# APRIL-ZJU/Ctrl-VIO

Hardware: AMD Instinct MI355X
Metric: sliding-window solves/sec (10 KF, 200 lm, 2000 IMU) (higher is better)
Workload: dtype f64; 1 GPU; config2: 10 KF / 200 landmarks / 2000 IMU sliding window (K = 24 knots, 814 reprojection blocks), <= 15 LM iterations (Ceres 1.14 trust region + projected line search); distinct_windows_per_gpu=64, streams_per_gpu=4, concurrent_solves_per_gpu=2

## Files before the change

### ctrl-vio_amd/csrc/factors.hpp

```cpp
#pragma once
#include "so3.hpp"

namespace ctv {

struct Knots4 {
  Q4 q[4];
  V3 p[4];
};

struct SegConst {
  V3 d[3];
  M3 JrI[3];
  CTV_DI M3 jri(int i) const { return JrI[i]; }
};
struct SegConstLazy {
  V3 d[3];
  const double *tab;
  CTV_DI M3 jri(int i) const {
    M3 J;
#pragma unroll
    for (int e = 0; e < 9; ++e) J.m[e] = tab[9 * i + e];
    return J;
  }
};
struct SegConstS {
  V3 d[3];
  M3 JrI[3];
  CTV_DI const M3 &jri(int i) const { return JrI[i]; }
};
CTV_DI void seg_const_lazy(const double *kd, const double *kjri, SegConstLazy &sc) {
#pragma unroll
  for (int i = 0; i < 3; ++i) sc.d[i] = mk(kd[3 * i], kd[3 * i + 1], kd[3 * i + 2]);
  sc.tab = kjri;
}
CTV_DI void seg_const(const Knots4 &k, SegConst &sc, bool want_jac) {
#pragma unroll
  for (int i = 0; i < 3; ++i) {
    sc.d[i] = so3_log(qmul(qconj(k.q[i]), k.q[i + 1]));
    if (want_jac) sc.JrI[i] = so3_Jr_inv(sc.d[i]);
  }
}

CTV_DI void knot_pair_const(const double *qa, const double *qb, double *d3, double *jri9) {
  const V3 dd = so3_log(qmul(qconj(qmk(qa[0], qa[1], qa[2], qa[3])), qmk(qb[0], qb[1], qb[2], qb[3])));
  d3[0] = dd.x; d3[1] = dd.y; d3[2] = dd.z;
  if (jri9) {
    const M3 J = so3_Jr_inv(mk(dd.x, dd.y, dd.z));
#pragma unroll
    for (int e = 0; e < 9; ++e) jri9[e] = J.m[e];
  }
}
CTV_DI void seg_const_load(const double *kd, const double *kjri, SegConst &sc, bool want_jac) {
#pragma unroll
  for (int i = 0; i < 3; ++i) {
    sc.d[i] = mk(kd[3 * i], kd[3 * i + 1], kd[3 * i + 2]);
    if (want_jac) {
#pragma unroll
      for (int e = 0; e < 9; ++e) sc.JrI[i].m[e] = kjri[9 * i + e];
    }
  }
}

struct ImuJac {
  M3 Jw[4], Ja[4];
  M3 Rinv_g;
  double lamA[4];
};

template <class SC> 
CTV_DI void imu_eval_core(const Knots4 &k, const SC &sc, double u, double idt, V3 gravity, const double bias[6],
                          const double gyro[3], const double acc[3], const double w[6], const M3 &RrefT, double r[6], bool want_jac, ImuJac &J) {
  double lamR[4], lamW[4];
  double (&lamA)[4] = J.lamA;
  basis<false, 2>(u, idt * idt, lamA);
  basis<true, 0>(u, 1.0, lamR);
  basis<true, 1>(u, idt, lamW);

  V3 accel = mk(0, 0, 0);
#pragma unroll
  for (int i = 0; i < 4; ++i) accel = accel + lamA[i] * k.p[i];

  Q4 Ainv[3], accq = qmk(0, 0, 0, 1);
  M3 Apost[4], JrK[3];
  Apost[3] = m3_id();
#pragma unroll
  for (int i = 2; i >= 0; --i) {
    const V3 nkd = (-lamR[i + 1]) * sc.d[i];
    Ainv[i] = so3_exp(nkd);
    accq = qmul_unit(accq, Ainv[i]);
    if (want_jac) { Apost[i] = q2R(accq); JrK[i] = so3_Jr(nkd); }
  }
  V3 om[4];
  om[0] = mk(0, 0, 0);
#pragma unroll
  for (int i = 0; i < 3; ++i) om[i + 1] = qrot(Ainv[i], om[i]) + lamW[i + 1] * sc.d[i];

  const Q4 Rinv_q = qmul_unit(accq, qconj(k.q[0]));
  const V3 ag = accel + gravity;
  const V3 a_pred = qrot(Rinv_q, ag);
  r[0] = w[0] * (om[3].x - (gyro[0] - bias[0]));
  r[1] = w[1] * (om[3].y - (gyro[1] - bias[1]));
  r[2] = w[2] * (om[3].z - (gyro[2] - bias[2]));
  r[3] = w[3] * (a_pred.x - (acc[0] - bias[3]));
  r[4] = w[4] * (a_pred.y - (acc[1] - bias[4]));
  r[5] = w[5] * (a_pred.z - (acc[2] - bias[5]));
  if (!want_jac) return;

  M3 (&Jw)[4] = J.Jw;
  M3 (&Ja)[4] = J.Ja;
#pragma unroll
  for (int i = 0; i < 4; ++i) { Jw[i] = m3_zero(); Ja[i] = m3_zero(); }
  {
    M3 dod = scale(Apost[1], lamW[1]);
#pragma unroll
    for (int i = 0; i < 3; ++i) {
      if (i > 0) dod = add(scale(mul(mul_hat(Apost[i], om[i]), JrK[i]), lamR[i + 1]), scale(Apost[i + 1], lamW[i + 1]));
      const M3 JrIi = sc.jri(i);
      Jw[i] = sub(Jw[i], mulT(dod, JrIi));
      Jw[i + 1] = add(Jw[i + 1], mul(dod, JrIi));
    }
  }
  const M3 Rinv = q2R(Rinv_q);
  J.Rinv_g = mul(Rinv, RrefT);
  {
    const M3 lhs = mul_hat(Rinv, ag);
    M3 Racc = q2R(k.q[0]);
    Ja[0] = add(Ja[0], mul(lhs, Racc));
#pragma unroll
    for (int i = 0; i < 3; ++i) {
      if (i > 0) Racc = mulT(Racc, q2R(Ainv[i - 1]));
      const M3 dad = scale(mul(mul(lhs, Racc), JrK[i]), lamR[i + 1]);
      const M3 JrIi = sc.jri(i);
      Ja[i] = sub(Ja[i], mulT(dad, JrIi));
      Ja[i + 1] = add(Ja[i + 1], mul(dad, JrIi));
    }
  }
}

CTV_DI void imu_row_gyro2(const M3 (&Jw)[4], const double w[6], const double r[6], int a, double out[16]) {
#pragma unroll
  for (int kk = 0; kk < 4; ++kk)
#pragma unroll
    for (int b = 0; b < 3; ++b) out[3 * kk + b] = w[a] * Jw[kk].m[3 * a + b];
  out[12] = out[13] = out[14] = 0.0;
  out[12 + a] = w[a];
  out[15] = r[a];
}

struct ImuMid3 {
  M3 Apost[3];
  M3 JrK[3];
  V3 om1, om2;
  V3 b[3];
  double lamR[4], lamW[4], lamA[4];
};
template <class SC> 
CTV_DI void imu_eval_values3(const double *gc, const SC &sc, double u, double idt, const double gyro[3], const double acc[3], const double w[6], double r[6], ImuMid3 &md) {
  basis<false, 2>(u, idt * idt, md.lamA);
  basis<true, 0>(u, 1.0, md.lamR);
  basis<true, 1>(u, idt, md.lamW);
  V3 ag = mk(gc[21], gc[22], gc[23]);
#pragma unroll
  for (int i = 1; i < 4; ++i) ag = ag + md.lamA[i] * mk(gc[3 * i], gc[3 * i + 1], gc[3 * i + 2]);
  Q4 Ainv[3], accq;
#pragma unroll
  for (int i = 2; i >= 0; --i) {
    const V3 nkd = (-md.lamR[i + 1]) * sc.d[i];
    Ainv[i] = so3_exp_small(nkd);
    accq = i == 2 ? Ainv[2] : qmul_unit(accq, Ainv[i]);
    md.Apost[i] = q2R(accq);
    md.JrK[i] = so3_Jr_small(nkd);
  }
  V3 om3;
  md.om1 = md.lamW[1] * sc.d[0];
  md.om2 = qrot(Ainv[1], md.om1) + md.lamW[2] * sc.d[1];
  om3 = qrot(Ainv[2], md.om2) + md.lamW[3] * sc.d[2];
  md.b[0] = mk(gc[12] * ag.x + gc[13] * ag.y + gc[14] * ag.z, gc[15] * ag.x + gc[16] * ag.y + gc[17] * ag.z,
                  gc[18] * ag.x + gc[19] * ag.y + gc[20] * ag.z);
  md.b[1] = qrot(Ainv[0], md.b[0]);
  md.b[2] = qrot(Ainv[1], md.b[1]);
  const V3 a_pred = qrot(Ainv[2], md.b[2]);
  r[0] = w[0] * (om3.x - (gyro[0] - gc[24]));
  r[1] = w[1] * (om3.y - (gyro[1] - gc[25]));
  r[2] = w[2] * (om3.z - (gyro[2] - gc[26]));
  r[3] = w[3] * (a_pred.x - (acc[0] - gc[27]));
  r[4] = w[4] * (a_pred.y - (acc[1] - gc[28]));
  r[5] = w[5] * (a_pred.z - (acc[2] - gc[29]));
}
template <class SC> CTV_DI void imu_apply_pair(const M3 &M, const SC &sc, int i, M3 &Ji, M3 &Ji1, bool first) {
  const M3 JrIi = sc.jri(i);
  const M3 A = mulT(M, JrIi), B = mul(M, JrIi);
#pragma unroll
  for (int e = 0; e < 9; ++e) { Ji.m[e] = first ? -A.m[e] : Ji.m[e] - A.m[e]; Ji1.m[e] = B.m[e]; }
}
template <class SC> CTV_DI void imu_jac_gyro3(const ImuMid3 &md, const SC &sc, M3 (&Jw)[4]) {
  imu_apply_pair(scale(md.Apost[1], md.lamW[1]), sc, 0, Jw[0], Jw[1], true);
  imu_apply_pair(add(scale(mul(mul_hat(md.Apost[1], md.om1), md.JrK[1]), md.lamR[2]), scale(md.Apost[2], md.lamW[2])), sc, 1, Jw[1], Jw[2], false);
  M3 dod = scale(mul(mul_hat(md.Apost[2], md.om2), md.JrK[2]), md.lamR[3]);
  dod.m[0] += md.lamW[3]; dod.m[4] += md.lamW[3]; dod.m[8] += md.lamW[3];
  imu_apply_pair(dod, sc, 2, Jw[2], Jw[3], false);
}
template <class SC> 
CTV_DI void imu_jac_accel3(const ImuMid3 &md, const SC &sc, const double *gc, M3 (&Ja)[4], M3 &Rinv_g) {
#pragma unroll
  for (int i = 0; i < 3; ++i)
#pragma unroll
    for (int j = 0; j < 3; ++j)
      Rinv_g.m[3 * i + j] = md.Apost[0].m[3 * i] * gc[12 + j] + md.Apost[0].m[3 * i + 1] * gc[15 + j] + md.Apost[0].m[3 * i + 2] * gc[18 + j];
  Ja[0] = mul_hat(md.Apost[0], md.b[0]);
#pragma unroll
  for (int i = 0; i < 3; ++i)
    imu_apply_pair(scale(mul(mul_hat(md.Apost[i], md.b[i]), md.JrK[i]), md.lamR[i + 1]), sc, i, Ja[i], Ja[i + 1], false);
}

CTV_DI void imu_row_accel3(const M3 (&Ja)[4], const double lamA[4], const M3 &Rinv_g, const double w[6], const double r[6], int a, double out[28]) {
#pragma unroll
  for (int kk = 0; kk < 4; ++kk)
#pragma unroll
    for (int b = 0; b < 3; ++b) {
      out[3 * kk + b] = w[3 + a] * Ja[kk].m[3 * a + b];
      out[16 + 3 * kk + b] = w[3 + a] * lamA[kk] * Rinv_g.m[3 * a + b];
    }
  out[12] = out[13] = out[14] = 0.0;
  out[12 + a] = w[3 + a];
  out[15] = r[3 + a];
}
template <class Sink> CTV_DI void imu_emit_cols(const ImuJac &J, const double w[6], Sink &sink) {
#pragma unroll
  for (int kk = 0; kk < 4; ++kk)
#pragma unroll
    for (int b = 0; b < 3; ++b) {
      double c6[6], p6[6];
#pragma unroll
      for (int a = 0; a < 3; ++a) {
        c6[a] = w[a] * J.Jw[kk].m[3 * a + b];
        c6[3 + a] = w[3 + a] * J.Ja[kk].m[3 * a + b];
        p6[a] = 0.0;
        p6[3 + a] = w[3 + a] * J.lamA[kk] * J.Rinv_g.m[3 * a + b];
      }
      sink.put_col(3 * kk + b, c6);
      sink.put_col(12 + 3 * kk + b, p6);
    }
#pragma unroll
  for (int a = 0; a < 3; ++a) {
    double g6[6] = {0.0, 0.0, 0.0, 0.0, 0.0, 0.0}, h6[6] = {0.0, 0.0, 0.0, 0.0, 0.0, 0.0};
    g6[a] = w[a];
    h6[3 + a] = w[3 + a];
    sink.put_col(24 + a, g6);
    sink.put_col(27 + a, h6);
  }
}
CTV_DI void imu_row_accel(const ImuJac &J, const double w[6], const double r[6], int a, double out[32]) {
#pragma unroll
  for (int kk = 0; kk < 4; ++kk)
#pragma unroll
    for (int b = 0; b < 3; ++b) {
      out[3 * kk + b] = w[3 + a] * J.Ja[kk].m[3 * a + b];
      out[12 + 3 * kk + b] = w[3 + a] * J.lamA[kk] * J.Rinv_g.m[3 * a + b];
    }
#pragma unroll
  for (int c = 24; c < 32; ++c) out[c] = 0.0;
  out[27 + a] = w[3 + a];
  out[30] = r[3 + a];
}
CTV_DI void imu_row_gyro(const ImuJac &J, const double w[6], const double r[6], int a, double out[16]) {
#pragma unroll
  for (int kk = 0; kk < 4; ++kk)
#pragma unroll
    for (int b = 0; b < 3; ++b) out[3 * kk + b] = w[a] * J.Jw[kk].m[3 * a + b];
  out[12] = out[13] = out[14] = 0.0;
  out[12 + a] = w[a];
  out[15] = r[a];
}

template <class Sink, class SC> 
CTV_DI void imu_eval(const Knots4 &k, const SC &sc, double u, double idt, V3 gravity, const double bias[6],
                     const double gyro[3], const double acc[3], const double w[6], const M3 &RrefT, double r[6], bool want_jac, Sink &sink) {
  ImuJac J;
  imu_eval_core<SC>(k, sc, u, idt, gravity, bias, gyro, acc, w, RrefT, r, want_jac, J);
  if (want_jac) imu_emit_cols(J, w, sink);
}

template <class SC, bool SMALL = false> CTV_DI Q4 eval_Rp(const Q4 q[4], const SC &sc, double u, M3 J[4], bool want_jac) {
  double c[4];
  basis<true, 0>(u, 1.0, c);
  Q4 accq = qmk(0, 0, 0, 1);
  M3 Apost[4], JrK[3];
  Apost[3] = m3_id();
#pragma unroll
  for (int i = 2; i >= 0; --i) {
    const V3 kd = c[i + 1] * sc.d[i];
    accq = qmul_unit(accq, so3_exp_sel<SMALL>(neg(kd)));
    if (want_jac) { JrK[i] = so3_Jr_sel<SMALL>(kd); Apost[i] = q2R(accq); }
  }
  const Q4 res = qmul_unit(q[0], qconj(accq));
  if (want_jac) {
    J[0] = Apost[0];
#pragma unroll
    for (int i = 0; i < 3; ++i) {
      const M3 Jh = scale(mul(Apost[i + 1], JrK[i]), c[i + 1]);
      J[i] = sub(J[i], mulT(Jh, sc.jri(i)));
      J[i + 1] = mul(Jh, sc.jri(i));
    }
  }
  return res;
}
template <class SC, bool SMALL = false> CTV_DI Q4 eval_RTp(const Q4 q[4], const SC &sc, double u, M3 J[4], bool want_jac) {
  double c[4];
  basis<true, 0>(u, 1.0, c);
  Q4 S[4];
  M3 JrK[3];
  S[0] = q[0];
#pragma unroll
  for (int i = 0; i < 3; ++i) {
    const V3 kd = c[i + 1] * sc.d[i];
    S[i + 1] = qmul_unit(S[i], so3_exp_sel<SMALL>(kd));
    if (want_jac) JrK[i] = so3_Jr_sel<SMALL>(neg(kd));
  }
  if (want_jac) {
    J[0] = q2R(S[0]);
#pragma unroll
    for (int i = 0; i < 3; ++i) {
      const M3 Jh = scale(mul(q2R(S[i]), JrK[i]), c[i + 1]);
      J[i] = sub(J[i], mulT(Jh, sc.jri(i)));
      J[i + 1] = mul(Jh, sc.jri(i));
    }
  }
  return qconj(S[3]);
}
template <class SC, bool SMALL = false> CTV_DI V3 eval_omega(const SC &sc, double u, double idt) {
  double c[4], dc[4];
  basis<true, 0>(u, 1.0, c);
  basis<true, 1>(u, idt, dc);
  V3 rv = dc[1] * sc.d[0];
#pragma unroll
  for (int i = 1; i < 3; ++i) rv = qrot(so3_exp_sel<SMALL>((-c[i + 1]) * sc.d[i]), rv) + dc[i + 1] * sc.d[i];
  return rv;
}
template <class SC> CTV_DI Q4 eval_R(const Q4 q[4], const SC &sc, double u) {
  double c[4];
  basis<true, 0>(u, 1.0, c);
  Q4 res = q[0];
#pragma unroll
  for (int i = 0; i < 3; ++i) res = qmul_unit(res, so3_exp(c[i + 1] * sc.d[i]));
  return res;
}

template <class SC> CTV_DI void pose_jac_T(const Q4 q[4], const SC &sc, double u, bool ext_on, Q4 q_SI, V3 p_SI, double *jt) {
  M3 J[4];
  const Q4 R = eval_Rp<SC>(q, sc, u, J, true);
  double c[4];
  basis<false, 0>(u, 1.0, c);
  M3 RSI = m3_id(), X = m3_zero();
  if (ext_on) { RSI = q2R(q_SI); X = scale(mul_hat(q2R(R), p_SI), -1.0); }
#pragma unroll
  for (int k = 0; k < 4; ++k) {
    const M3 B = mul(X, J[k]);
#pragma unroll
    for (int cc = 0; cc < 3; ++cc)
#pragma unroll
      for (int a = 0; a < 3; ++a) {
        jt[(6 * k + cc) * 6 + a] = ext_on ? RSI.m[a] * J[k].m[cc] + RSI.m[3 + a] * J[k].m[3 + cc] + RSI.m[6 + a] * J[k].m[6 + cc] : J[k].m[3 * a + cc];
        jt[(6 * k + cc) * 6 + 3 + a] = ext_on ? B.m[3 * a + cc] : 0.0;
        jt[(6 * k + 3 + cc) * 6 + a] = 0.0;
        jt[(6 * k + 3 + cc) * 6 + 3 + a] = a == cc ? c[k] : 0.0;
      }
  }
}

template <class SC> CTV_DI void nav_jac_T(const Q4 q[4], const SC &sc, double u, double idt, double *jt, double cv[4]) {
  pose_jac_T(q, sc, u, false, qmk(0.0, 0.0, 0.0, 1.0), mk(0.0, 0.0, 0.0), jt);
  basis<false, 1>(u, idt, cv);
}

CTV_DI void rel_pose_jac_T(Q4 q_a, V3 p_a, Q4 q_b, V3 p_b, double *jt_a, double *jt_b, Q4 &q_ab, V3 &p_ab) {
  q_ab = qmul(qconj(q_a), q_b);
  const M3 Ra = q2R(q_a), Rab = q2R(q_ab);
  const V3 d = p_b - p_a;
// ... 256 lines not shown
```

### ctrl-vio_amd/csrc/kernels_imu.hpp

```cpp
#pragma once

namespace ctv {

template <class T, int N> struct alignas(N * sizeof(T)) VecN { T v[N]; };

typedef double f64x4 __attribute__((ext_vector_type(4)));

__device__ __forceinline__ void imu_zero_share(const Dev &d, int mode, const ImuGroup &grp, int gidx, int zero_mode) {
  if (!zero_mode) return;
  const int w = grp.win, lane = threadIdx.x;
  const WinMeta &m = d.wins[w];
  const int tg = lin_target(d.lm[w], mode);
  double *Hpp = d.HppS[tg] + m.H0, *g = d.gS[tg] + m.u0;
  const int nH = m.P * m.ldh, first = (m.vis_lds && zero_mode == 1) ? 6 * m.K * m.ldh : 0;
  const int gi = gidx - m.grp0, per = (((nH - first) / 2 + m.ngrp - 1) / m.ngrp) * 2;
  const int lo = first + gi * per, hi = min(lo + per, nH);
  for (int i = lo + 2 * lane; i < hi; i += 128) *reinterpret_cast<double2 *>(Hpp + i) = double2{0.0, 0.0};
  if (gi == 0) {
    for (int i = lane; i < m.P; i += 64) g[i] = 0.0;
    if (lane == 0) { if (mode == LIN_SPEC) d.lm[w].cand_gmax_bits = 0ull; else d.lm[w].gmax_bits = 0ull; }
  }
}

__device__ __forceinline__ void imu_linearize_f64_body(const Dev &d, int mode, double *A , int gidx, int zero_mode) {
  const ImuGroup grp = d.groups[gidx];
  const int w = grp.win;
  if (!lin_run(d.lm[w], mode)) return;
  const bool jac = !lin_cost_only(d.lm[w], mode, d.prm);
  if (jac) imu_zero_share(d, mode, grp, gidx, zero_mode);
  const WinMeta &m = d.wins[w];
  const int lane = threadIdx.x, q4 = lane >> 4, l15 = lane & 15;
  const bool at_cand = mode == LIN_SPEC;
  double csum = 0.0;
  const double *s_quat = at_cand ? d.cquat : d.quat, *s_pos = at_cand ? d.cpos : d.pos, *s_bias = at_cand ? d.cbias : d.bias;
  Knots4 k;
  LocalFrame lf;
  lf.init(s_quat, s_pos, m.knot0 + grp.s);
  lf.load(s_quat, s_pos, m.knot0 + grp.s, k);
  const M3 RrefT = lf.RrefT();
  SegConstLazy sc;
  seg_const_lazy(d.lkd + 3 * (m.knot0 + grp.s), d.kjri + 9 * (m.knot0 + grp.s), sc);
  double bias[6], wgt[6];
  const double *bp = s_bias + 6 * (m.bias0 + grp.bias);
#pragma unroll
  for (int i = 0; i < 6; ++i) { bias[i] = bp[i]; wgt[i] = m.imu_w[i]; }
  const V3 grav = lf.rotate(m.gravity);
  const double idt = m.inv_dt;
  f64x4 acc00 = {0.0, 0.0, 0.0, 0.0}, acc10 = {0.0, 0.0, 0.0, 0.0}, acc11 = {0.0, 0.0, 0.0, 0.0}, gacc = {0.0, 0.0, 0.0, 0.0};
  const size_t Mt = (size_t)d.Mtot;
  if (!jac) {
    for (int c0 = 0; c0 < grp.count; c0 += 64) {
      const bool live = c0 + lane < grp.count;
      const int idx = m.imu0 + grp.start + min(c0 + lane, grp.count - 1);
      double gy[3], ac[3], r[6], wl[6];
#pragma unroll
      for (int i = 0; i < 3; ++i) { gy[i] = d.imu_meas[(size_t)i * Mt + idx]; ac[i] = d.imu_meas[(size_t)(3 + i) * Mt + idx]; }
#pragma unroll
      for (int i = 0; i < 6; ++i) wl[i] = live ? wgt[i] : 0.0;
      ImuJac J;
      imu_eval_core(k, sc, d.imu_u[idx], idt, grav, bias, gy, ac, wl, RrefT, r, false, J);
#pragma unroll
      for (int i = 0; i < 6; ++i) csum += 0.5 * r[i] * r[i];
    }
#pragma unroll
    for (int off = 32; off > 0; off >>= 1) csum += __shfl_xor(csum, off);
    if (lane == 0) d.imu_cost[gidx] = csum;
    return;
  }
  for (int c0 = 0; c0 < grp.count; c0 += 64) {
    const int nval = min(64, grp.count - c0);
    const bool live = lane < nval;
    const int idx = m.imu0 + grp.start + min(c0 + lane, grp.count - 1);
    double gy[3], ac[3], r[6];
#pragma unroll
    for (int i = 0; i < 3; ++i) { gy[i] = d.imu_meas[(size_t)i * Mt + idx]; ac[i] = d.imu_meas[(size_t)(3 + i) * Mt + idx]; }
    double wl[6];
#pragma unroll
    for (int i = 0; i < 6; ++i) wl[i] = live ? wgt[i] : 0.0;
    const int kmax = (nval + 3) & ~3;
    ImuJac J;
    imu_eval_core(k, sc, d.imu_u[idx], idt, grav, bias, gy, ac, wl, RrefT, r, true, J);
#pragma unroll
    for (int i = 0; i < 6; ++i) csum += 0.5 * r[i] * r[i];
#pragma unroll
    for (int a = 0; a < 3; ++a) {
      double row[32];
      imu_row_accel(J, wl, r, a, row);
      __builtin_amdgcn_wave_barrier();
#pragma unroll
      for (int c = 0; c < 32; ++c) A[lane * 33 + c] = row[c];
      lds_wave_sync();
      for (int k0 = 0; k0 < kmax; k0 += 4) {
        const double lo = A[(k0 + q4) * 33 + l15], hi = A[(k0 + q4) * 33 + 16 + l15];
        acc00 = __builtin_amdgcn_mfma_f64_16x16x4f64(lo, lo, acc00, 0, 0, 0);
        acc10 = __builtin_amdgcn_mfma_f64_16x16x4f64(hi, lo, acc10, 0, 0, 0);
        acc11 = __builtin_amdgcn_mfma_f64_16x16x4f64(hi, hi, acc11, 0, 0, 0);
      }
    }
#pragma unroll
    for (int a = 0; a < 3; ++a) {
      double row[16];
      imu_row_gyro(J, wl, r, a, row);
      __builtin_amdgcn_wave_barrier();
#pragma unroll
      for (int c = 0; c < 16; ++c) A[lane * 17 + c] = row[c];
      lds_wave_sync();
      for (int k0 = 0; k0 < kmax; k0 += 4) {
        const double v = A[(k0 + q4) * 17 + l15];
        gacc = __builtin_amdgcn_mfma_f64_16x16x4f64(v, v, gacc, 0, 0, 0);
      }
    }
  }
#pragma unroll
  for (int off = 32; off > 0; off >>= 1) csum += __shfl_xor(csum, off);
  if (lane == 0) d.imu_cost[gidx] = csum;
  __builtin_amdgcn_wave_barrier();
#pragma unroll
  for (int r = 0; r < 4; ++r) {
    const int row = q4 + 4 * r, col = l15;
    A[row * 32 + col] = acc00[r];
    A[(16 + row) * 32 + 16 + col] = acc11[r];
    A[(16 + row) * 32 + col] = acc10[r];
    A[col * 32 + 16 + row] = acc10[r];
  }
  lds_wave_sync();
  {
    const int tc = l15 < 12 ? l15 : (l15 < 15 ? l15 + 12 : 30);
#pragma unroll
    for (int r = 0; r < 4; ++r) {
      const int grow = q4 + 4 * r;
      const int tr = grow < 12 ? grow : (grow < 15 ? grow + 12 : 30);
      A[tr * 32 + tc] += gacc[r];
    }
  }
  lds_wave_sync();
  double *tile = d.imu_tiles + (size_t)gidx * 1024;
#pragma unroll
  for (int i = 0; i < 16; ++i) tile[i * 64 + lane] = A[i * 64 + lane];
}

typedef double f64x2 __attribute__((ext_vector_type(2)));
__device__ __forceinline__ void imu_chain_gyro(const double *A, int q4, int l15, int kmax, f64x4 &gacc) {
  unsigned addr = (unsigned)(size_t)(A + q4 * 17 + l15);
  double v0, v1;
  asm volatile("ds_read_b64 %0, %1" : "=v"(v0) : "v"(addr));
  for (int k0 = 0; k0 < kmax; k0 += 8) {
    asm volatile("ds_read_b64 %0, %1 offset:544" : "=v"(v1) : "v"(addr));
    asm volatile("s_waitcnt lgkmcnt(1)" : "+v"(v0));
    gacc = __builtin_amdgcn_mfma_f64_16x16x4f64(v0, v0, gacc, 0, 0, 0);
    addr += 8 * 17 * 8;
    asm volatile("ds_read_b64 %0, %1" : "=v"(v0) : "v"(addr));
    asm volatile("s_waitcnt lgkmcnt(1)" : "+v"(v1));
    gacc = __builtin_amdgcn_mfma_f64_16x16x4f64(v1, v1, gacc, 0, 0, 0);
  }
  asm volatile("s_waitcnt lgkmcnt(0)" : "+v"(v0));
}
__device__ __forceinline__ void imu_chain_accel(const double *A, int q4, int l15, int kmax, f64x4 &acc00, f64x4 &acc10) {
  unsigned addr = (unsigned)(size_t)(A + q4 * 33 + l15);
  f64x2 o0, o1;
  asm volatile("ds_read2_b64 %0, %1 offset1:16" : "=v"(o0) : "v"(addr));
  for (int k0 = 0; k0 < kmax; k0 += 8) {
    asm volatile("ds_read2_b64 %0, %1 offset0:132 offset1:148" : "=v"(o1) : "v"(addr));
    asm volatile("s_waitcnt lgkmcnt(1)" : "+v"(o0));
    acc00 = __builtin_amdgcn_mfma_f64_16x16x4f64(o0[0], o0[0], acc00, 0, 0, 0);
    acc10 = __builtin_amdgcn_mfma_f64_16x16x4f64(o0[1], o0[0], acc10, 0, 0, 0);
    addr += 8 * 33 * 8;
    asm volatile("ds_read2_b64 %0, %1 offset1:16" : "=v"(o0) : "v"(addr));
    asm volatile("s_waitcnt lgkmcnt(1)" : "+v"(o1));
    acc00 = __builtin_amdgcn_mfma_f64_16x16x4f64(o1[0], o1[0], acc00, 0, 0, 0);
    acc10 = __builtin_amdgcn_mfma_f64_16x16x4f64(o1[1], o1[0], acc10, 0, 0, 0);
  }
  asm volatile("s_waitcnt lgkmcnt(0)" : "+v"(o0));
}

__device__ __forceinline__ bool imu_fast_pred(const double kd[9], const double *imu_w) {
  double mx = 0.0;
#pragma unroll
  for (int i = 0; i < 3; ++i) mx = fmax(mx, __fma_rn(kd[3 * i + 2], kd[3 * i + 2], __fma_rn(kd[3 * i + 1], kd[3 * i + 1], __dmul_rn(kd[3 * i], kd[3 * i]))));
  return mx < 0.25 && imu_w[3] == imu_w[4] && imu_w[3] == imu_w[5];
}
struct ImuPre { double pc, kq; int fl; };
__device__ __forceinline__ void imu_prefetch(const Dev &d, int mode, const ImuGroup &g, int lane, ImuPre &o) {
  const bool at_cand = mode == LIN_SPEC;
  const double *s_quat = at_cand ? d.cquat : d.quat, *s_pos = at_cand ? d.cpos : d.pos, *s_bias = at_cand ? d.cbias : d.bias;
  const WinMeta &m = d.wins[g.win];
  const Lm &lm = d.lm[g.win];
  const double *kd = d.lkd + 3 * g.kabs, *kj = d.kjri + 9 * g.kabs;
  const double *q = s_quat + 4 * g.kabs, *pp = s_pos + 3 * g.kabs, *bp = s_bias + 6 * g.babs;
  o.pc = *(lane < 9 ? kd + lane : kj + (min(lane, 35) - 9));
  const double *src = lane < 4 ? q + lane : lane < 16 ? pp + (lane - 4) : lane < 21 ? q : lane < 24 ? m.gravity + (lane - 21)
                      : lane < 30 ? bp + (lane - 24) : lane < 36 ? m.imu_w + (lane - 30) : &m.inv_dt;
  o.kq = *src;
  const int32_t *fp = lane == 0 ? &lm.status : lane == 1 ? &lm.step_valid : lane == 2 ? &lm.iter : &lm.ls_active;
  o.fl = *fp;
}
__device__ __forceinline__ void imu_linearize_f64_fast(const Dev &d, int mode, double *A , int g0, int stride, int zero_mode) {
  const int lane = threadIdx.x, q4 = lane >> 4, l15 = lane & 15;
  const size_t Mt = (size_t)d.Mtot;
  int gidx = g0;
  ImuGroup grp = d.groups[gidx];
  ImuPre cur;
  imu_prefetch(d, mode, grp, lane, cur);
  double gyn[3], acn[3], un;
  {
    const int idx = grp.iabs + min(lane, grp.count - 1);
#pragma unroll
    for (int i = 0; i < 3; ++i) { gyn[i] = d.imu_meas[(size_t)i * Mt + idx]; acn[i] = d.imu_meas[(size_t)(3 + i) * Mt + idx]; }
    un = d.imu_u[idx];
  }
  bool has_next = gidx + stride < d.Gtot;
  ImuGroup grpn = d.groups[has_next ? gidx + stride : gidx];
  for (;;) {
  const bool has_next2 = has_next && gidx + 2 * stride < d.Gtot;
  const ImuGroup grpn2 = d.groups[has_next2 ? gidx + 2 * stride : gidx];
  ImuPre nxt;
  imu_prefetch(d, mode, grpn, lane, nxt);
  bool nmeas = false;
  do {
  const int w = grp.win;
  const int base = grp.iabs;
  SegConstS sc;
#pragma unroll
  for (int i = 0; i < 3; ++i) {
    sc.d[i] = mk(readlane_d(cur.pc, 3 * i), readlane_d(cur.pc, 3 * i + 1), readlane_d(cur.pc, 3 * i + 2));
#pragma unroll
    for (int e = 0; e < 9; ++e) sc.JrI[i].m[e] = readlane_d(cur.pc, 9 + 9 * i + e);
  }
  const int f_status = __builtin_amdgcn_readlane(cur.fl, 0), f_valid = __builtin_amdgcn_readlane(cur.fl, 1), f_iter = __builtin_amdgcn_readlane(cur.fl, 2),
            f_ls = __builtin_amdgcn_readlane(cur.fl, 3);
  if (!(f_status == 0 && (mode != LIN_SPEC || f_valid != 0))) break;
  const bool jac = !(mode == COST_AT_X || (mode == LIN_SPEC && f_iter >= d.prm.max_iters && f_ls == 0));
  {
    const double kd9[9] = {sc.d[0].x, sc.d[0].y, sc.d[0].z, sc.d[1].x, sc.d[1].y, sc.d[1].z, sc.d[2].x, sc.d[2].y, sc.d[2].z};
    const double w6[6] = {0.0, 0.0, 0.0, readlane_d(cur.kq, 33), readlane_d(cur.kq, 34), readlane_d(cur.kq, 35)};
    if (!imu_fast_pred(kd9, w6)) break;
  }
  long long *dbg = (d.dbg && gidx == 5000 && jac) ? d.dbg + 64 : nullptr;
  int dbi = 0;
  CTV_STAMP(dbg, dbi, 16, lane == 0);
  double *gc = A + 72 * 33;
  {
    double gcv = cur.kq;
    const M3 R0 = q2R(qmk(readlane_d(cur.kq, 0), readlane_d(cur.kq, 1), readlane_d(cur.kq, 2), readlane_d(cur.kq, 3)));
    const double pk = __shfl(cur.kq, 4 + min(lane, 11)), p0 = __shfl(cur.kq, 4 + min(lane, 11) % 3);
    if (lane < 12) gcv = pk - p0;
    else if (lane < 21) {
      const int e = lane - 12, src = 3 * (e % 3) + e / 3;
#pragma unroll
      for (int i = 0; i < 9; ++i) gcv = src == i ? R0.m[i] : gcv;
    }
    __builtin_amdgcn_wave_barrier();
    if (lane < 36) gc[lane] = gcv;
    lds_wave_sync();
  }
  const double idt = readlane_d(cur.kq, 36);
  double csum = 0.0;
  if (!jac) {
    for (int c0 = 0; c0 < grp.count; c0 += 64) {
      const bool live = c0 + lane < grp.count;
      const int idx = base + min(c0 + lane, grp.count - 1);
      double gy[3], ac[3], r[6], wl[6];
#pragma unroll
      for (int i = 0; i < 3; ++i) { gy[i] = d.imu_meas[(size_t)i * Mt + idx]; ac[i] = d.imu_meas[(size_t)(3 + i) * Mt + idx]; }
#pragma unroll
      for (int i = 0; i < 6; ++i) wl[i] = live ? gc[30 + i] : 0.0;
      ImuMid3 md;
      imu_eval_values3(gc, sc, d.imu_u[idx], idt, gy, ac, wl, r, md);
#pragma unroll
      for (int i = 0; i < 6; ++i) csum += 0.5 * r[i] * r[i];
    }
#pragma unroll
    for (int off = 32; off > 0; off >>= 1) csum += __shfl_xor(csum, off);
    if (lane == 0) d.imu_cost[gidx] = csum;
    break;
  }
  f64x4 acc00 = {0.0, 0.0, 0.0, 0.0}, acc10 = {0.0, 0.0, 0.0, 0.0}, gacc = {0.0, 0.0, 0.0, 0.0};
  double spp[10] = {0.0, 0.0, 0.0, 0.0, 0.0, 0.0, 0.0, 0.0, 0.0, 0.0};
  for (int c0 = 0; c0 < grp.count; c0 += 64) {
    CTV_STAMP(dbg, dbi, 16, lane == 0, csum);
    const int nval = min(64, grp.count - c0);
    const bool live = lane < nval;
    double gy[3], ac[3], r[6];
#pragma unroll
    for (int i = 0; i < 3; ++i) { gy[i] = gyn[i]; ac[i] = acn[i]; }
    const double u = un;
    {
      const bool last = c0 + 64 >= grp.count;
      const int idx = (last && has_next) ? grpn.iabs + min(lane, grpn.count - 1) : base + min(c0 + 64 + lane, grp.count - 1);
      nmeas = last;
#pragma unroll
      for (int i = 0; i < 3; ++i) { gyn[i] = d.imu_meas[(size_t)i * Mt + idx]; acn[i] = d.imu_meas[(size_t)(3 + i) * Mt + idx]; }
      un = d.imu_u[idx];
    }
    double wl[6];
#pragma unroll
    for (int i = 0; i < 6; ++i) wl[i] = live ? gc[30 + i] : 0.0;
    const int kmax = (nval + 3) & ~3;
    ImuMid3 md;
    imu_eval_values3(gc, sc, u, idt, gy, ac, wl, r, md);
#pragma unroll
    for (int i = 0; i < 6; ++i) csum += 0.5 * r[i] * r[i];
    CTV_STAMP(dbg, dbi, 16, lane == 0, csum);
    {
      M3 Jw[4];
      imu_jac_gyro3(md, sc, Jw);
      CTV_STAMP(dbg, dbi, 16, lane == 0, Jw[3].m[8]);
#pragma unroll
      for (int a = 0; a < 3; ++a) {
        double row[16];
        imu_row_gyro2(Jw, wl, r, a, row);
        __builtin_amdgcn_wave_barrier();
#pragma unroll
        for (int c = 0; c < 16; ++c) A[lane * 17 + c] = row[c];
        lds_wave_sync();
        imu_chain_gyro(A, q4, l15, kmax, gacc);
      }
    }
    CTV_STAMP(dbg, dbi, 16, lane == 0, gacc[0]);
    {
      M3 Ja[4], Rinv_g;
      imu_jac_accel3(md, sc, gc, Ja, Rinv_g);
      CTV_STAMP(dbg, dbi, 16, lane == 0, Ja[3].m[8] + Rinv_g.m[8]);
      {
        double la[4];
#pragma unroll
        for (int kk = 0; kk < 4; ++kk) la[kk] = wl[3] * md.lamA[kk];
        int e = 0;
#pragma unroll
        for (int ka = 0; ka < 4; ++ka)
#pragma unroll
          for (int kb = 0; kb <= ka; ++kb) { spp[e] += la[ka] * la[kb]; ++e; }
      }
#pragma unroll
      for (int a = 0; a < 3; ++a) {
        double row[28];
        imu_row_accel3(Ja, md.lamA, Rinv_g, wl, r, a, row);
        __builtin_amdgcn_wave_barrier();
#pragma unroll
        for (int c = 0; c < 28; ++c) A[lane * 33 + c] = row[c];
        lds_wave_sync();
        imu_chain_accel(A, q4, l15, kmax, acc00, acc10);
      }
    }
  }
  CTV_STAMP(dbg, dbi, 16, lane == 0, acc00[0] + acc10[0]);
  __builtin_amdgcn_wave_barrier();
#pragma unroll
  for (int i = 0; i < 16; ++i) A[i * 64 + lane] = 0.0;
  {
    double *S = A + 1024;
#pragma unroll
    for (int e = 0; e < 10; ++e) S[e * 64 + lane] = spp[e];
    S[10 * 64 + lane] = csum;
    lds_wave_sync();
    const int e = min(lane >> 2, 10), part = lane & 3;
    double t = 0.0;
#pragma unroll
    for (int i = 0; i < 16; ++i) t += S[e * 64 + part * 16 + i];
    t += __shfl_xor(t, 1);
    t += __shfl_xor(t, 2);
    __builtin_amdgcn_wave_barrier();
    if (lane < 40 && part == 0) S[704 + e] = t;
    if (lane == 40) d.imu_cost[gidx] = t;
  }
  lds_wave_sync();
  {
    const int c0 = l15 < 12 ? l15 : (l15 < 15 ? l15 + 15 : 30);
    const int cg = l15 < 12 ? l15 : (l15 < 15 ? l15 + 12 : 30);
    const bool cb = l15 >= 12 && l15 < 15;
#pragma unroll
    for (int r = 0; r < 4; ++r) {
      const int t = q4 + 4 * r;
      const int r0 = t < 12 ? t : (t < 15 ? t + 15 : 30), rg = t < 12 ? t : (t < 15 ? t + 12 : 30);
      const bool shared = !cb && !(t >= 12 && t < 15);
      A[r0 * 32 + c0] = shared ? acc00[r] + gacc[r] : acc00[r];
      if (!shared) A[rg * 32 + cg] = gacc[r];
      if (t < 12) { A[(12 + t) * 32 + c0] = acc10[r]; A[c0 * 32 + 12 + t] = acc10[r]; }
    }
    const int ka = lane / 12, kb = (lane / 3) & 3, b = lane % 3;
    const int hi = max(ka, kb), lo = min(ka, kb);
    if (lane < 48) A[(12 + 3 * ka + b) * 32 + 12 + 3 * kb + b] = A[1024 + 704 + hi * (hi + 1) / 2 + lo];
  }
  lds_wave_sync();
  double *tile = d.imu_tiles + (size_t)gidx * 1024;
#pragma unroll
  for (int i = 0; i < 8; ++i)
    *reinterpret_cast<double2 *>(tile + i * 128 + 2 * lane) = *reinterpret_cast<const double2 *>(A + i * 128 + 2 * lane);
  imu_zero_share(d, mode, grp, gidx, zero_mode);
  CTV_STAMP(dbg, dbi, 16, lane == 0);
  } while (false);
  if (!has_next) break;
  lds_wave_sync();
  if (!nmeas) {
    const int idx = grpn.iabs + min(lane, grpn.count - 1);
#pragma unroll
    for (int i = 0; i < 3; ++i) { gyn[i] = d.imu_meas[(size_t)i * Mt + idx]; acn[i] = d.imu_meas[(size_t)(3 + i) * Mt + idx]; }
    un = d.imu_u[idx];
  }
  gidx += stride;
  grp = grpn; grpn = grpn2; cur = nxt;
  has_next = has_next2;
  }
}

__device__ __forceinline__ bool imu_group_fast(const Dev &d, int gidx) {
  const ImuGroup grp = d.groups[gidx];
  const double *kd = d.lkd + 3 * grp.kabs;
  const double kd9[9] = {kd[0], kd[1], kd[2], kd[3], kd[4], kd[5], kd[6], kd[7], kd[8]};
  return imu_fast_pred(kd9, d.wins[grp.win].imu_w);
}
__global__ __launch_bounds__(64) __attribute__((amdgpu_waves_per_eu(1, 1))) void k_imu_linearize_f64(Dev d, int mode, int general_only, int zero_mode) {
  extern __shared__ __attribute__((aligned(32))) unsigned char smraw[];
  if (!general_only) imu_linearize_f64_fast(d, mode, reinterpret_cast<double *>(smraw), blockIdx.x, gridDim.x, zero_mode);
}
__device__ __forceinline__ void imu_rest_body(const Dev &d, int mode, int general_only, int zero_mode, unsigned char *smraw , int w) {
  const WinMeta &m = d.wins[w];
  for (int g0 = 0; g0 < m.ngrp; g0 += 64) {
    const int gl = g0 + (int)threadIdx.x;
    const bool need = gl < m.ngrp && (general_only || !imu_group_fast(d, m.grp0 + gl));
    unsigned long long todo = __ballot(need);
    while (todo) {
      const int b = __ffsll((long long)todo) - 1;
      todo &= todo - 1;
      imu_linearize_f64_body(d, mode, reinterpret_cast<double *>(smraw), m.grp0 + g0 + b, zero_mode);
      lds_wave_sync();
    }
  }
}
__global__ __launch_bounds__(64) __attribute__((amdgpu_waves_per_eu(1, 1))) void k_imu_linearize_rest(Dev d, int mode, int general_only, int zero_mode) {
  extern __shared__ __attribute__((aligned(32))) unsigned char smraw[];
  imu_rest_body(d, mode, general_only, zero_mode, smraw, blockIdx.x);
}

__device__ __forceinline__ int imu_knot_major_to_col(int j) {
  const int k = j / 6, c = j - 6 * k;
  return c < 3 ? 3 * k + c : 9 + 3 * k + c;
}
__device__ __forceinline__ void imu_bias_rows_accumulate(const Dev &d, const WinMeta &m, double *Hpp, double *g) {
  const int lane = threadIdx.x & 63, wave = threadIdx.x >> 6, ldh = m.ldh;
  const int nmine = (m.ngrp - wave + 3) >> 2;
  for (int i = lane; i < 195 * nmine; i += 64) {
    const int q = i / 195, t = i - 195 * q, gi = m.grp0 + wave + 4 * q;
    const ImuGroup grp = d.groups[gi];
    const double *tile = d.imu_tiles + (size_t)gi * 1024;
    const int B = 6 * grp.s, R = 6 * m.K + 6 * grp.bias;
    if (t < 144) {
      const int r = t / 24, j = t - 24 * r;
      atomicAdd(&Hpp[(long long)(R + r) * ldh + B + j], tile[(24 + r) * 32 + imu_knot_major_to_col(j)]);
    } else if (t < 165) {
      const int e = t - 144;
      const int r = e < 1 ? 0 : e < 3 ? 1 : e < 6 ? 2 : e < 10 ? 3 : e < 15 ? 4 : 5, c = e - r * (r + 1) / 2;
      atomicAdd(&Hpp[(long long)(R + r) * ldh + R + c], tile[(24 + r) * 32 + 24 + c]);
    } else {
      const int j = t - 165;
      atomicAdd(&g[j < 24 ? B + j : R + j - 24], tile[30 * 32 + (j < 24 ? imu_knot_major_to_col(j) : j)]);
    }
  }
}

__device__ __forceinline__ void assemble_imu_window(const Dev &d, int mode, int w, double *band ) {
  if (!lin_run(d.lm[w], mode) || lin_cost_only(d.lm[w], mode, d.prm)) return;
  const WinMeta &m = d.wins[w];
  const int K = m.K, ldh = m.ldh, tg = lin_target(d.lm[w], mode);
  double *Hpp = d.HppS[tg] + m.H0, *g = d.gS[tg] + m.u0;
  if (m.vis_lds) {
    imu_bias_rows_accumulate(d, m, Hpp, g);
    return;
  }
  if (band) {
    const int nb = 144 * K;
    for (int i = threadIdx.x; i < nb; i += 256) band[i] = 0.0;
    __syncthreads();
    for (int i = threadIdx.x; i < 300 * m.ngrp; i += 256) {
      const int gi = i / 300, t = i - 300 * gi;
      int a = (int)((sqrtf(8.0f * (float)t + 1.0f) - 1.0f) * 0.5f);
      a += ((a + 1) * (a + 2) / 2 <= t) ? 1 : 0;
      a -= (a * (a + 1) / 2 > t) ? 1 : 0;
      const int b = t - a * (a + 1) / 2;
      const ImuGroup grp = d.groups[m.grp0 + gi];
      const double v = d.imu_tiles[(size_t)(m.grp0 + gi) * 1024 + a * 32 + b];
      int ga = imu_col(a, grp.s, K, grp.bias), gb = imu_col(b, grp.s, K, grp.bias);
      if (ga < gb) { const int tmp = ga; ga = gb; gb = tmp; }
      const int k1 = ga / 6, k2 = gb / 6;
      atomicAdd(&band[((k2 * 4 + (k1 - k2)) * 6 + (ga - 6 * k1)) * 6 + (gb - 6 * k2)], v);
    }
    __syncthreads();
    for (int i = threadIdx.x; i < nb; i += 256) {
      const double v = band[i];
      if (v == 0.0) continue;
      const int r2 = i % 6, r1 = (i / 6) % 6, dk = (i / 36) % 4, k2 = i / 144;
      const int ga = 6 * (k2 + dk) + r1, gb = 6 * k2 + r2;
      atomicAdd(&Hpp[(long long)ga * ldh + gb], v);
    }
    imu_bias_rows_accumulate(d, m, Hpp, g);
    return;
  }
  for (int i = threadIdx.x; i < 31 * 30 * m.ngrp; i += 256) {
    const int gi = i / 930, e = i - 930 * gi;
    const ImuGroup grp = d.groups[m.grp0 + gi];
    const double *tile = d.imu_tiles + (size_t)(m.grp0 + gi) * 1024;
    const int b = e / 30, a = e % 30;
    const double v = tile[a * 32 + b];
    const int ga = imu_col(a, grp.s, K, grp.bias);
    if (b == 30) { atomicAdd(&g[ga], v); continue; }
    const int gb = imu_col(b, grp.s, K, grp.bias);
    if (ga >= gb) atomicAdd(&Hpp[(long long)ga * ldh + gb], v);
  }
}

}
```

Baseline: 50190 solves/s.

## Factor IMU Jacobian through shared pair-log transform and world-frame accel rows

Restructures the per-measurement IMU Jacobian so the knot-rotation chain rule (JrI pair terms) is applied once per group, as a 16x16 transform T on the accumulated Gram matrices, instead of per measurement. Accelerometer rows are rotated into a world frame, so the position block collapses to scalar lamA weights multiplied against a small 16-wide row using 4x4x4 MFMAs rather than a 28-wide row with a second 16x16 accumulator. This cuts per-sample ALU work and LDS traffic. In exchange it adds extra MFMA post-processing, more LDS scratch, and some numerical reordering in f64.

```diff
diff --git a/ctrl-vio_amd/csrc/factors.hpp b/ctrl-vio_amd/csrc/factors.hpp
--- a/ctrl-vio_amd/csrc/factors.hpp
+++ b/ctrl-vio_amd/csrc/factors.hpp
@@ -135,16 +135,6 @@
       Ja[i + 1] = add(Ja[i + 1], mul(dad, JrIi));
     }
   }
-}
-
-CTV_DI void imu_row_gyro2(const M3 (&Jw)[4], const double w[6], const double r[6], int a, double out[16]) {
-#pragma unroll
-  for (int kk = 0; kk < 4; ++kk)
-#pragma unroll
-    for (int b = 0; b < 3; ++b) out[3 * kk + b] = w[a] * Jw[kk].m[3 * a + b];
-  out[12] = out[13] = out[14] = 0.0;
-  out[12 + a] = w[a];
-  out[15] = r[a];
 }
 
 struct ImuMid3 {
@@ -187,43 +177,64 @@
   r[4] = w[4] * (a_pred.y - (acc[1] - gc[28]));
   r[5] = w[5] * (a_pred.z - (acc[2] - gc[29]));
 }
-template <class SC> CTV_DI void imu_apply_pair(const M3 &M, const SC &sc, int i, M3 &Ji, M3 &Ji1, bool first) {
-  const M3 JrIi = sc.jri(i);
-  const M3 A = mulT(M, JrIi), B = mul(M, JrIi);
-#pragma unroll
-  for (int e = 0; e < 9; ++e) { Ji.m[e] = first ? -A.m[e] : Ji.m[e] - A.m[e]; Ji1.m[e] = B.m[e]; }
-}
-template <class SC> CTV_DI void imu_jac_gyro3(const ImuMid3 &md, const SC &sc, M3 (&Jw)[4]) {
-  imu_apply_pair(scale(md.Apost[1], md.lamW[1]), sc, 0, Jw[0], Jw[1], true);
-  imu_apply_pair(add(scale(mul(mul_hat(md.Apost[1], md.om1), md.JrK[1]), md.lamR[2]), scale(md.Apost[2], md.lamW[2])), sc, 1, Jw[1], Jw[2], false);
-  M3 dod = scale(mul(mul_hat(md.Apost[2], md.om2), md.JrK[2]), md.lamR[3]);
-  dod.m[0] += md.lamW[3]; dod.m[4] += md.lamW[3]; dod.m[8] += md.lamW[3];
-  imu_apply_pair(dod, sc, 2, Jw[2], Jw[3], false);
-}
-template <class SC> 
-CTV_DI void imu_jac_accel3(const ImuMid3 &md, const SC &sc, const double *gc, M3 (&Ja)[4], M3 &Rinv_g) {
+CTV_DI void imu_pairlog_slots(int i, int a, int b, int &plus, int &minus) {
+  plus = (3 + 3 * i + a) * 16 + 3 * (i + 1) + b;
+  minus = (3 + 3 * i + b) * 16 + 3 * i + a;
+}
+template <class SC> CTV_DI void imu_pairlog_T(const SC &sc, double T[256]) {
+  for (int e = 0; e < 256; ++e) T[e] = 0.0;
+  for (int k = 0; k < 16; ++k)
+    if (k < 3 || k >= 12) T[17 * k] = 1.0;
+  for (int i = 0; i < 3; ++i) {
+    const M3 J = sc.jri(i);
+    for (int a = 0; a < 3; ++a)
+      for (int b = 0; b < 3; ++b) {
+        int plus, minus;
+        imu_pairlog_slots(i, a, b, plus, minus);
+        T[plus] = J.m[3 * a + b];
+        T[minus] = -J.m[3 * a + b];
+      }
+  }
+}
+CTV_DI void imu_pair_gyro3(const ImuMid3 &md, M3 (&M)[3]) {
+  M[0] = scale(md.Apost[1], md.lamW[1]);
+  M[1] = add(scale(mul(mul_hat(md.Apost[1], md.om1), md.JrK[1]), md.lamR[2]), scale(md.Apost[2], md.lamW[2]));
+  M[2] = scale(mul(mul_hat(md.Apost[2], md.om2), md.JrK[2]), md.lamR[3]);
+  M[2].m[0] += md.lamW[3]; M[2].m[4] += md.lamW[3]; M[2].m[8] += md.lamW[3];
+}
+CTV_DI void imu_row_gyro_pl(const M3 (&M)[3], const double w[6], const double r[6], int a, double out[16]) {
+  out[0] = out[1] = out[2] = 0.0;
 #pragma unroll
   for (int i = 0; i < 3; ++i)
 #pragma unroll
-    for (int j = 0; j < 3; ++j)
-      Rinv_g.m[3 * i + j] = md.Apost[0].m[3 * i] * gc[12 + j] + md.Apost[0].m[3 * i + 1] * gc[15 + j] + md.Apost[0].m[3 * i + 2] * gc[18 + j];
-  Ja[0] = mul_hat(md.Apost[0], md.b[0]);
+    for (int b = 0; b < 3; ++b) out[3 + 3 * i + b] = w[a] * M[i].m[3 * a + b];
+  out[12] = out[13] = out[14] = 0.0;
+  out[12 + a] = w[a];
+  out[15] = r[a];
+}
+CTV_DI void imu_world_accel3(const ImuMid3 &md, const double *gc, const double w[6], const double r[6], double Y[3][16]) {
+  M3 R0;
 #pragma unroll
   for (int i = 0; i < 3; ++i)
-    imu_apply_pair(scale(mul(mul_hat(md.Apost[i], md.b[i]), md.JrK[i]), md.lamR[i + 1]), sc, i, Ja[i], Ja[i + 1], false);
-}
-
-CTV_DI void imu_row_accel3(const M3 (&Ja)[4], const double lamA[4], const M3 &Rinv_g, const double w[6], const double r[6], int a, double out[28]) {
-#pragma unroll
-  for (int kk = 0; kk < 4; ++kk)
-#pragma unroll
-    for (int b = 0; b < 3; ++b) {
-      out[3 * kk + b] = w[3 + a] * Ja[kk].m[3 * a + b];
-      out[16 + 3 * kk + b] = w[3 + a] * lamA[kk] * Rinv_g.m[3 * a + b];
-    }
-  out[12] = out[13] = out[14] = 0.0;
-  out[12 + a] = w[3 + a];
-  out[15] = r[3 + a];
+#pragma unroll
+    for (int j = 0; j < 3; ++j) R0.m[3 * i + j] = gc[12 + 3 * j + i];
+  const M3 Rs = mulT(R0, md.Apost[0]), wRs = scale(Rs, w[3]);
+  M3 blk[4];
+  blk[0] = mul_hat(R0, w[3] * md.b[0]);
+  blk[1] = mul(scale(blk[0], md.lamR[1]), md.JrK[0]);
+#pragma unroll
+  for (int i = 1; i < 3; ++i) blk[i + 1] = mul(Rs, scale(mul(mul_hat(md.Apost[i], md.b[i]), md.JrK[i]), w[3] * md.lamR[i + 1]));
+#pragma unroll
+  for (int a = 0; a < 3; ++a) {
+#pragma unroll
+    for (int kk = 0; kk < 4; ++kk)
+#pragma unroll
+      for (int b = 0; b < 3; ++b) Y[a][3 * kk + b] = blk[kk].m[3 * a + b];
+#pragma unroll
+    for (int b = 0; b < 3; ++b) Y[a][12 + b] = wRs.m[3 * a + b];
+  }
+#pragma unroll
+  for (int a = 0; a < 3; ++a) Y[a][15] = Rs.m[3 * a] * r[3] + Rs.m[3 * a + 1] * r[4] + Rs.m[3 * a + 2] * r[5];
 }
 template <class Sink> CTV_DI void imu_emit_cols(const ImuJac &J, const double w[6], Sink &sink) {
 #pragma unroll
diff --git a/ctrl-vio_amd/csrc/kernels_imu.hpp b/ctrl-vio_amd/csrc/kernels_imu.hpp
--- a/ctrl-vio_amd/csrc/kernels_imu.hpp
+++ b/ctrl-vio_amd/csrc/kernels_imu.hpp
@@ -139,7 +139,6 @@
   for (int i = 0; i < 16; ++i) tile[i * 64 + lane] = A[i * 64 + lane];
 }
 
-typedef double f64x2 __attribute__((ext_vector_type(2)));
 __device__ __forceinline__ void imu_chain_gyro(const double *A, int q4, int l15, int kmax, f64x4 &gacc) {
   unsigned addr = (unsigned)(size_t)(A + q4 * 17 + l15);
   double v0, v1;
@@ -155,22 +154,26 @@
   }
   asm volatile("s_waitcnt lgkmcnt(0)" : "+v"(v0));
 }
-__device__ __forceinline__ void imu_chain_accel(const double *A, int q4, int l15, int kmax, f64x4 &acc00, f64x4 &acc10) {
-  unsigned addr = (unsigned)(size_t)(A + q4 * 33 + l15);
-  f64x2 o0, o1;
-  asm volatile("ds_read2_b64 %0, %1 offset1:16" : "=v"(o0) : "v"(addr));
+__device__ __forceinline__ void imu_chain_world(const double *A, const double *L, int q4, int l15, int kmax, f64x4 &acc00, double &x) {
+  unsigned addr = (unsigned)(size_t)(A + q4 * 17 + l15), laddr = (unsigned)(size_t)(L + q4 * 4 + (l15 & 3));
+  double v0, v1, a0, a1;
+  asm volatile("ds_read_b64 %0, %1" : "=v"(v0) : "v"(addr));
+  asm volatile("ds_read_b64 %0, %1" : "=v"(a0) : "v"(laddr));
   for (int k0 = 0; k0 < kmax; k0 += 8) {
-    asm volatile("ds_read2_b64 %0, %1 offset0:132 offset1:148" : "=v"(o1) : "v"(addr));
-    asm volatile("s_waitcnt lgkmcnt(1)" : "+v"(o0));
-    acc00 = __builtin_amdgcn_mfma_f64_16x16x4f64(o0[0], o0[0], acc00, 0, 0, 0);
-    acc10 = __builtin_amdgcn_mfma_f64_16x16x4f64(o0[1], o0[0], acc10, 0, 0, 0);
-    addr += 8 * 33 * 8;
-    asm volatile("ds_read2_b64 %0, %1 offset1:16" : "=v"(o0) : "v"(addr));
-    asm volatile("s_waitcnt lgkmcnt(1)" : "+v"(o1));
-    acc00 = __builtin_amdgcn_mfma_f64_16x16x4f64(o1[0], o1[0], acc00, 0, 0, 0);
-    acc10 = __builtin_amdgcn_mfma_f64_16x16x4f64(o1[1], o1[0], acc10, 0, 0, 0);
-  }
-  asm volatile("s_waitcnt lgkmcnt(0)" : "+v"(o0));
+    asm volatile("ds_read_b64 %0, %1 offset:544" : "=v"(v1) : "v"(addr));
+    asm volatile("ds_read_b64 %0, %1 offset:128" : "=v"(a1) : "v"(laddr));
+    asm volatile("s_waitcnt lgkmcnt(2)" : "+v"(v0), "+v"(a0));
+    acc00 = __builtin_amdgcn_mfma_f64_16x16x4f64(v0, v0, acc00, 0, 0, 0);
+    x = __builtin_amdgcn_mfma_f64_4x4x4f64(a0, v0, x, 0, 0, 0);
+    addr += 8 * 17 * 8;
+    laddr += 8 * 4 * 8;
+    asm volatile("ds_read_b64 %0, %1" : "=v"(v0) : "v"(addr));
+    asm volatile("ds_read_b64 %0, %1" : "=v"(a0) : "v"(laddr));
+    asm volatile("s_waitcnt lgkmcnt(2)" : "+v"(v1), "+v"(a1));
+    acc00 = __builtin_amdgcn_mfma_f64_16x16x4f64(v1, v1, acc00, 0, 0, 0);
+    x = __builtin_amdgcn_mfma_f64_4x4x4f64(a1, v1, x, 0, 0, 0);
+  }
+  asm volatile("s_waitcnt lgkmcnt(0)" : "+v"(v0), "+v"(a0));
 }
 
 __device__ __forceinline__ bool imu_fast_pred(const double kd[9], const double *imu_w) {
@@ -221,11 +224,7 @@
   const int base = grp.iabs;
   SegConstS sc;
 #pragma unroll
-  for (int i = 0; i < 3; ++i) {
-    sc.d[i] = mk(readlane_d(cur.pc, 3 * i), readlane_d(cur.pc, 3 * i + 1), readlane_d(cur.pc, 3 * i + 2));
-#pragma unroll
-    for (int e = 0; e < 9; ++e) sc.JrI[i].m[e] = readlane_d(cur.pc, 9 + 9 * i + e);
-  }
+  for (int i = 0; i < 3; ++i) sc.d[i] = mk(readlane_d(cur.pc, 3 * i), readlane_d(cur.pc, 3 * i + 1), readlane_d(cur.pc, 3 * i + 2));
   const int f_status = __builtin_amdgcn_readlane(cur.fl, 0), f_valid = __builtin_amdgcn_readlane(cur.fl, 1), f_iter = __builtin_amdgcn_readlane(cur.fl, 2),
             f_ls = __builtin_amdgcn_readlane(cur.fl, 3);
   if (!(f_status == 0 && (mode != LIN_SPEC || f_valid != 0))) break;
@@ -274,8 +273,10 @@
     if (lane == 0) d.imu_cost[gidx] = csum;
     break;
   }
-  f64x4 acc00 = {0.0, 0.0, 0.0, 0.0}, acc10 = {0.0, 0.0, 0.0, 0.0}, gacc = {0.0, 0.0, 0.0, 0.0};
+  f64x4 acc00 = {0.0, 0.0, 0.0, 0.0}, gacc = {0.0, 0.0, 0.0, 0.0};
+  double xpos[3] = {0.0, 0.0, 0.0};
   double spp[10] = {0.0, 0.0, 0.0, 0.0, 0.0, 0.0, 0.0, 0.0, 0.0, 0.0};
+  double *Lw = A + 1280;
   for (int c0 = 0; c0 < grp.count; c0 += 64) {
     CTV_STAMP(dbg, dbi, 16, lane == 0, csum);
     const int nval = min(64, grp.count - c0);
@@ -302,13 +303,13 @@
     for (int i = 0; i < 6; ++i) csum += 0.5 * r[i] * r[i];
     CTV_STAMP(dbg, dbi, 16, lane == 0, csum);
     {
-      M3 Jw[4];
-      imu_jac_gyro3(md, sc, Jw);
-      CTV_STAMP(dbg, dbi, 16, lane == 0, Jw[3].m[8]);
+      M3 Mw[3];
+      imu_pair_gyro3(md, Mw);
+      CTV_STAMP(dbg, dbi, 16, lane == 0, Mw[2].m[8]);
 #pragma unroll
       for (int a = 0; a < 3; ++a) {
         double row[16];
-        imu_row_gyro2(Jw, wl, r, a, row);
+        imu_row_gyro_pl(Mw, wl, r, a, row);
         __builtin_amdgcn_wave_barrier();
 #pragma unroll
         for (int c = 0; c < 16; ++c) A[lane * 17 + c] = row[c];
@@ -318,13 +319,13 @@
     }
     CTV_STAMP(dbg, dbi, 16, lane == 0, gacc[0]);
     {
-      M3 Ja[4], Rinv_g;
-      imu_jac_accel3(md, sc, gc, Ja, Rinv_g);
-      CTV_STAMP(dbg, dbi, 16, lane == 0, Ja[3].m[8] + Rinv_g.m[8]);
+      double Y[3][16];
+      imu_world_accel3(md, gc, wl, r, Y);
+      CTV_STAMP(dbg, dbi, 16, lane == 0, Y[2][15]);
+      double la[4];
+#pragma unroll
+      for (int kk = 0; kk < 4; ++kk) la[kk] = wl[3] * md.lamA[kk];
       {
-        double la[4];
-#pragma unroll
-        for (int kk = 0; kk < 4; ++kk) la[kk] = wl[3] * md.lamA[kk];
         int e = 0;
 #pragma unroll
         for (int ka = 0; ka < 4; ++ka)
@@ -333,22 +334,28 @@
       }
 #pragma unroll
       for (int a = 0; a < 3; ++a) {
-        double row[28];
-        imu_row_accel3(Ja, md.lamA, Rinv_g, wl, r, a, row);
         __builtin_amdgcn_wave_barrier();
 #pragma unroll
-        for (int c = 0; c < 28; ++c) A[lane * 33 + c] = row[c];
+        for (int c = 0; c < 16; ++c) A[lane * 17 + c] = Y[a][c];
+        if (a == 0) {
+#pragma unroll
+          for (int kk = 0; kk < 4; ++kk) Lw[lane * 4 + kk] = la[kk];
+        }
         lds_wave_sync();
-        imu_chain_accel(A, q4, l15, kmax, acc00, acc10);
+        imu_chain_world(A, Lw, q4, l15, kmax, acc00, xpos[a]);
       }
     }
   }
-  CTV_STAMP(dbg, dbi, 16, lane == 0, acc00[0] + acc10[0]);
+  CTV_STAMP(dbg, dbi, 16, lane == 0, acc00[0] + xpos[0]);
   __builtin_amdgcn_wave_barrier();
 #pragma unroll
   for (int i = 0; i < 16; ++i) A[i * 64 + lane] = 0.0;
+  double *S = A + 1024, *Tp = A + 1792, *Xs = A + 2048;
+#pragma unroll
+  for (int i = 0; i < 4; ++i) Tp[i * 64 + lane] = 0.0;
+#pragma unroll
+  for (int b = 0; b < 3; ++b) Xs[(3 * q4 + b) * 17 + l15] = xpos[b];
   {
-    double *S = A + 1024;
 #pragma unroll
     for (int e = 0; e < 10; ++e) S[e * 64 + lane] = spp[e];
     S[10 * 64 + lane] = csum;
@@ -362,9 +369,36 @@
     __builtin_amdgcn_wave_barrier();
     if (lane < 40 && part == 0) S[704 + e] = t;
     if (lane == 40) d.imu_cost[gidx] = t;
+    if (lane >= 9 && lane < 36) {
+      const int i = (lane - 9) / 9, ab = (lane - 9) % 9;
+      int plus, minus;
+      imu_pairlog_slots(i, ab / 3, ab % 3, plus, minus);
+      Tp[plus] = cur.pc;
+      Tp[minus] = -cur.pc;
+    }
+    if (lane < 3 || (lane >= 12 && lane < 16)) Tp[17 * lane] = 1.0;
   }
   lds_wave_sync();
   {
+    double Tr[4], Xa[4];
+#pragma unroll
+    for (int r = 0; r < 4; ++r) {
+      Tr[r] = Tp[(q4 + 4 * r) * 16 + l15];
+      Xa[r] = Xs[min(l15, 11) * 17 + q4 + 4 * r];
+      Xa[r] = l15 < 12 ? Xa[r] : 0.0;
+    }
+    f64x4 zg = {0.0, 0.0, 0.0, 0.0}, za = {0.0, 0.0, 0.0, 0.0}, hg = {0.0, 0.0, 0.0, 0.0}, ha = {0.0, 0.0, 0.0, 0.0}, hx = {0.0, 0.0, 0.0, 0.0};
+#pragma unroll
+    for (int r = 0; r < 4; ++r) {
+      zg = __builtin_amdgcn_mfma_f64_16x16x4f64(gacc[r], Tr[r], zg, 0, 0, 0);
+      za = __builtin_amdgcn_mfma_f64_16x16x4f64(acc00[r], Tr[r], za, 0, 0, 0);
+      hx = __builtin_amdgcn_mfma_f64_16x16x4f64(Xa[r], Tr[r], hx, 0, 0, 0);
+    }
+#pragma unroll
+    for (int r = 0; r < 4; ++r) {
+      hg = __builtin_amdgcn_mfma_f64_16x16x4f64(Tr[r], zg[r], hg, 0, 0, 0);
+      ha = __builtin_amdgcn_mfma_f64_16x16x4f64(Tr[r], za[r], ha, 0, 0, 0);
+    }
     const int c0 = l15 < 12 ? l15 : (l15 < 15 ? l15 + 15 : 30);
     const int cg = l15 < 12 ? l15 : (l15 < 15 ? l15 + 12 : 30);
     const bool cb = l15 >= 12 && l15 < 15;
@@ -373,13 +407,17 @@
       const int t = q4 + 4 * r;
       const int r0 = t < 12 ? t : (t < 15 ? t + 15 : 30), rg = t < 12 ? t : (t < 15 ? t + 12 : 30);
       const bool shared = !cb && !(t >= 12 && t < 15);
-      A[r0 * 32 + c0] = shared ? acc00[r] + gacc[r] : acc00[r];
-      if (!shared) A[rg * 32 + cg] = gacc[r];
-      if (t < 12) { A[(12 + t) * 32 + c0] = acc10[r]; A[c0 * 32 + 12 + t] = acc10[r]; }
+      if (t >= l15) {
+        const double v = shared ? ha[r] + hg[r] : ha[r];
+        A[r0 * 32 + c0] = v;
+        A[c0 * 32 + r0] = v;
+        if (!shared) { A[rg * 32 + cg] = hg[r]; A[cg * 32 + rg] = hg[r]; }
+      }
+      if (t < 12) { A[(12 + t) * 32 + c0] = hx[r]; A[c0 * 32 + 12 + t] = hx[r]; }
     }
     const int ka = lane / 12, kb = (lane / 3) & 3, b = lane % 3;
     const int hi = max(ka, kb), lo = min(ka, kb);
-    if (lane < 48) A[(12 + 3 * ka + b) * 32 + 12 + 3 * kb + b] = A[1024 + 704 + hi * (hi + 1) / 2 + lo];
+    if (lane < 48) A[(12 + 3 * ka + b) * 32 + 12 + 3 * kb + b] = S[704 + hi * (hi + 1) / 2 + lo];
   }
   lds_wave_sync();
   double *tile = d.imu_tiles + (size_t)gidx * 1024;
```

Result: faster. 52030 solves/s, median of 6 (+3.7%).
